# sjpark0905/DNA-LDPC-codes

Measured on AMD Instinct MI355X. Metric: decoded codewords/sec (n=18432, m=2048, 50 BP iters) at 1/2/4/8 GPUs; % HBM roofline, higher is better.
Workload: dtype f64; 1 GPU; bsc-p0.02-100k-per-gpu-bp50; code=decode_n18432_m2048_final.pchk (8,72)-regular, E=147456, input=int8 channel codes in HBM + table code*ln49 (LR = host exp), batch_per_gpu=100000, global_batch=100000, max_iter=50, algo=bp, parallelism=dp1 (contiguous codeword shards, no collective), resident_per_pass=192, group_tiles=3, nontemporal_d=False, continuous=True, resident_pool=True, syndrome_split=False

## Files before the change

dna-ldpc-codes_amd/csrc/engine.hip:

```cpp
#include <hip/hip_ext.h>
#include <hip/hip_runtime.h>

#include <algorithm>
#include <cmath>
#include <cstdio>
#include <cstdlib>
#include <cstring>
#include <thread>
#include <type_traits>
#include <utility>

#include "engine.hpp"
#include "kernels.hpp"
#include "kernels_int.hpp"
#include "encode_kernels.hpp"

namespace ldpc {

static_assert(kTile == dev::TILE && kMsaRecPlanes == dev::MSA_REC_PLANES && kMsaErShift == dev::MSA_ER_SHIFT,
              "engine_plan.hpp restates the kernels' layout constants");
constexpr int kProbes = 4;

static thread_local std::string g_err;
void set_error(const std::string& msg) { g_err = msg; }
// ... 203 lines not shown
int LanePool::check_fault()
{
    if (!h_fault) return LDPC_OK;
    volatile unsigned long long* w = h_fault.get();
    std::string msg;
    for (int k = 1; k < dev::kFaultWords; k++) {
        const unsigned long long v = w[k];
        if (!(v & dev::kFaultTag)) continue;
        w[k] = 0ull;
        if (!msg.empty()) continue;
        int64_t idx = (int64_t)(v & dev::kFaultIndex);
        if (idx & (int64_t)(1ull << 47)) idx -= (int64_t)(1ull << 48);
        if (k == dev::kFaultSchedule)
            msg = "device schedule fault: the code fill of tile " + std::to_string(-1 - idx) +
                  " found live or finished lanes";
        else if (k == dev::kFaultIters)
            msg = "device lane bookkeeping fault: codeword index " + std::to_string(idx) +
                  " out of range for the iteration count / valid flag access";
        else
            msg = "device lane bookkeeping fault: pool slot or codeword index " + std::to_string(idx) +
                  " out of range for " + (k == dev::kFaultOutput ? "a finished codeword's hard bits / posterior" : "a refill's input row");
    }
    if (msg.empty()) return LDPC_OK;
    set_error(msg + " (skipped; the decode's outputs are incomplete)");
    return LDPC_ERR_DEVICE;
}

void LanePool::clear_faults()
{
    volatile unsigned long long* w = h_fault.get();
    for (int k = 1; w && k < dev::kFaultWords; k++) w[k] = 0ull;
}

Engine::~Engine()
{
    if (device >= 0) (void)hipSetDevice(device);
    if (stream) (void)hipStreamSynchronize(stream.get());
}

static double* msa_rec(double* scratch) { return scratch; }
static uint16_t* msa_meta(double* scratch, int64_t tiles, int32_t M)
{
    return reinterpret_cast<uint16_t*>(scratch + (size_t)tiles * M * dev::MSA_REC_PLANES * dev::TILE);
}

template <typename F>
static void with_bools(F&& f)
{
    f();
}
template <typename F, typename... Bs>
static void with_bools(F&& f, bool b, Bs... rest)
{
    if (b) with_bools([&](auto... cs) { f(std::true_type{}, cs...); }, rest...);
    else with_bools([&](auto... cs) { f(std::false_type{}, cs...); }, rest...);
}
template <int... Vs, typename F, typename... Bs>
static bool dispatch(int v, std::integer_sequence<int, Vs...>, F&& f, Bs... bs)
{
    return ((v == Vs && (with_bools([&](auto... cs) { f(std::integral_constant<int, Vs>{}, cs...); }, bs...), true)) || ...);
}

int Engine::init(const HostGraph* graph, int dev, int algorithm, int64_t chunk, const ldpc_schedule* schedule,
                 bool resolved)
{
    g = graph;
    device = dev;
    algo = algorithm;
    if (resolved && schedule && (schedule->flags_set & kResolved)) {
        sched = *schedule;
        sched.pool_tiles = std::max(sched.pool_tiles, 0);
        sched.poll_every = std::max(sched.poll_every, 1);
        sched.syn_blocks = std::min(std::max(sched.syn_blocks, 1), 256);
    } else {
        sched = resolve_schedule(schedule);
    }
    if (algo < LDPC_ALGO_BP || algo > LDPC_ALGO_GALLAGER_B2) { set_error("unknown algorithm"); return LDPC_ERR_ARG; }
    int rc;
    if ((rc = select_device("engine", dev)) || (rc = make_stream(stream))) return rc;
    size_t fr = 0, tot = 0;
    if (chunk <= 0) LDPC_HIP(hipMemGetInfo(&fr, &tot));
    p = plan_engine(*g, algo, chunk, sched, fr);
    if (p.error) { set_error(p.error); return LDPC_ERR_ARG; }

    if ((rc = dg.build(*g, p.msa_c))) return rc;
    if (p.cont && (rc = lp.build(p, g->N))) return rc;
    const size_t E = (size_t)std::max<int64_t>(g->E, 1), cap = (size_t)p.cap, tiles = (size_t)p.cap_tiles, N = (size_t)g->N;
    if ((rc = dev_alloc(v2c, cap * E))) return rc;
    if (!p.res && (rc = dev_alloc(c2v_buf, p.c2v_bytes / sizeof(double)))) return rc;
    if ((rc = dev_alloc(prior, cap * N)) || (p.msa_c && (rc = dev_alloc(d_sgn, cap * N))) ||
        (rc = dev_alloc(hard, tiles * N)) || (rc = dev_alloc(active, tiles)) || (rc = dev_alloc(iters, cap)) ||
        (rc = dev_alloc(valid, cap)))
        return rc;
    if (algo < LDPC_ALGO_QMSA && (p.res || p.group_tiles < p.cap_tiles)) return probe(kProbes);
    return LDPC_OK;
}

int32_t Engine::flags() const
{
    return (p.nt_d ? LDPC_SCHED_NONTEMPORAL : 0) | (p.cont ? LDPC_SCHED_CONTINUOUS : 0) |
           (p.msa_c ? LDPC_SCHED_MSA_COMPRESSED : 0) | (p.res ? LDPC_SCHED_RESIDENT : 0) |
           (p.syn_blocks > 0 ? LDPC_SCHED_SPLIT_SYNDROME : 0) | (p.first_fp ? LDPC_SCHED_FIRST_FROM_PRIOR : 0) |
           (p.handover ? LDPC_SCHED_HANDOVER : 0) | (p.fuse_block >= 0 ? LDPC_SCHED_FUSE_ROW_BLOCK : 0) |
           (sched.flags & (LDPC_SCHED_LR_TABLE | LDPC_SCHED_DEBUG_NO_DRAIN | LDPC_SCHED_DEBUG_BAD_LANE));
}

int Engine::probe(int probes)
{
    dev_ptr<double>& pool = p.res ? v2c : c2v_buf;
    std::vector<dev_ptr<double>> cand;
    cand.push_back(std::move(pool));
    size_t best = 0;
    const int rc = time_candidates(probes, cand, &best);
    pool = std::move(cand[best]);
    return rc;
}

int Engine::time_candidates(int probes, std::vector<dev_ptr<double>>& cand, size_t* best)
{
    const size_t E = (size_t)std::max<int64_t>(g->E, 1);
    const size_t bytes = p.res ? (size_t)p.cap * E * sizeof(double) : p.c2v_bytes;
    const unsigned gt = (unsigned)(p.res ? p.cap_tiles : std::min<int64_t>(p.group_tiles, p.cap_tiles));
    hipStream_t s = stream.get();
    LDPC_HIP(hipMemsetAsync((p.res ? cand[0] : v2c).get(), 0, (size_t)gt * 64 * E * sizeof(double), s));
    LDPC_HIP(hipMemsetAsync(prior.get(), 0, (size_t)gt * 64 * g->N * sizeof(double), s));
    LDPC_HIP(hipMemsetAsync(active.get(), 0xff, (size_t)gt * sizeof(uint64_t), s));
    if (d_sgn) LDPC_HIP(hipMemsetAsync(d_sgn.get(), 0, (size_t)gt * 64 * g->N, s));
    for (int i = 1; i < probes; i++) {
        void* c = nullptr;
        if (hipMalloc(&c, bytes) != hipSuccess) { (void)hipGetLastError(); break; }
        cand.emplace_back(static_cast<double*>(c));
    }
    for (auto& c : cand) LDPC_HIP(hipMemsetAsync(c.get(), 0, bytes, s));
    Event e0, e1;
    int rc;
    if ((rc = make_event(e0, hipEventDefault)) || (rc = make_event(e1, hipEventDefault))) return rc;
    float best_ms = 1e30f;
    for (size_t c = 0; c < cand.size(); c++) {
        if (p.res) std::swap(v2c, cand[c]);
        float ms = 0;
        rc = time_steps((p.res ? v2c : cand[c]).get(), gt, e0.get(), e1.get(), &ms);
        if (p.res) std::swap(v2c, cand[c]);
        if (rc) return rc;
        if (ms < best_ms) { best_ms = ms; *best = c; }
    }
    return LDPC_OK;
}

int Engine::time_steps(double* pool, unsigned gt, hipEvent_t e0, hipEvent_t e1, float* ms)
{
    int rc;
    for (int rep = 0; rep < 5; rep++) {
        if (rep == 1) LDPC_HIP(hipEventRecord(e0, stream.get()));
        if ((rc = launch_check(pool, 0, gt, nullptr, true))) return rc;
        if ((rc = launch_var(pool, 0, gt, nullptr, dev::Refill{}, true))) return rc;
    }
    LDPC_HIP(hipEventRecord(e1, stream.get()));
    LDPC_HIP(hipEventSynchronize(e1));
    LDPC_HIP(hipEventElapsedTime(ms, e0, e1));
    return LDPC_OK;
}

int Engine::launch_check(double* scratch, int64_t t0, unsigned gt, const dev::ResStep* rstep, bool timing)
{
    using namespace dev;
    const int32_t M = g->M;
    const int64_t E = g->E;
    const bool reg72 = g->regular_dc && g->dc_max == 72;
    const dim3 grid((M + 3) / 4, gt), blk(256);
    const bool msa = algo == LDPC_ALGO_MSA;
    const int kc = timing ? K_UNCOUNTED : K_CHECK;
    int rc = LDPC_OK;
    if (rstep && !reg72) {
        const int cb = gen_bucket(g->dc_max, CheckBuckets{});
        if (!p.res || scratch != v2c.get() || t0 != 0 || !cb) { set_error("resident check: bad state"); return LDPC_ERR_ARG; }
        dispatch(cb, CheckBuckets{}, [&](auto D, auto MSA) {
            rc = launch(kc, (k_check_gr_res<MSA(), D()>), grid, blk, v2c, dg.row_ptr, M, E, *rstep);
        }, msa);
        return rc;
    }
    if (rstep) {
        if (!p.res || p.msa_c || scratch != v2c.get()) { set_error("resident check: bad state"); return LDPC_ERR_ARG; }
        if (msa) return launch(kc, (k_check_msa<72, false, true>), grid, blk, v2c, v2c, active, M, E, t0, *rstep);
        if (p.fuse_block >= 0) {
            if (t0 != 0) { set_error("resident check: bad state"); return LDPC_ERR_ARG; }
            const int32_t Q = M / 8;
            return launch(kc, (k_check_bp_skip<72>), grid, blk, v2c, v2c, M, E, p.fuse_block * Q, (p.fuse_block + 1) * Q,
                          *rstep);
        }
        return launch(kc, (k_check_bp<72, false, true>), grid, blk, v2c, v2c, active, M, E, t0, *rstep);
    }
    if (p.msa_c) {
        const dim3 g1((unsigned)((M + 3) / 4) * gt);
        with_bools([&](auto NT) {
            rc = launch(kc, (k_check_msa_c<72, NT()>), g1, blk, v2c, msa_rec(scratch), msa_meta(scratch, p.c2v_tiles, M),
                        active, dg.row_pos, M, E, t0, gt);
        }, p.nt_d);
        return rc;
    }
    if (reg72) {
        with_bools([&](auto NT) {
            if (msa) rc = launch(kc, (k_check_msa<72, NT(), false>), grid, blk, v2c, scratch, active, M, E, t0, ResStep{});
            else rc = launch(kc, (k_check_bp<72, NT(), false>), grid, blk, v2c, scratch, active, M, E, t0, ResStep{});
        }, p.nt_d);
        return rc;
    }
    const bool bp = algo == LDPC_ALGO_BP;
    const bool in_regs = dispatch(gen_bucket(g->dc_max, CheckBuckets{}), CheckBuckets{}, [&](auto D, auto MSA) {
        rc = launch(kc, k_check_gr<MSA(), D()>, grid, blk, v2c, scratch, active, dg.row_ptr, M, E, t0);
    }, !bp);
    if (!in_regs && bp) rc = launch(kc, k_check_bp_gen, grid, blk, v2c, scratch, active, dg.row_ptr, M, E, t0);
    else if (!in_regs) rc = launch(kc, k_check_msa_gen, grid, blk, v2c, scratch, active, dg.row_ptr, M, E, t0);
    return rc;
}

int Engine::var_cpw_for(const dev::Refill& rf) const
{
    if (p.var_cpw > 0) return p.var_cpw;
    return (rf.fresh && rf.in_code && (p.res || p.msa_c)) ? kDefaultVarCpwCoded : kDefaultVarCpw;
}

int Engine::launch_var(double* scratch, int64_t t0, unsigned gt, double* pt, const dev::Refill& rf, bool timing)
{
    using namespace dev;
    const int32_t N = g->N, M = g->M;
    const int64_t E = g->E;
    const bool reg8 = g->regular_dv && g->dv_max == 8;
    const bool cnt = rf.fresh != nullptr;
    const bool pc = cnt && rf.in_code != nullptr;
    const bool inplace = scratch == v2c.get();
    const int kc = timing ? K_UNCOUNTED : K_VAR;
    int rc = LDPC_OK;
    bool ok = true;
    if (p.msa_c) {
        int cpw = std::min(var_cpw_for(rf), 4);
        if (N % (4 * cpw) != 0) cpw = 1;
        const unsigned nb = gt * (unsigned)(N / (4 * cpw));
        const double* rec = msa_rec(scratch);
        const uint16_t* meta = msa_meta(scratch, p.c2v_tiles, M);
        ok = dispatch(cpw, std::integer_sequence<int, 1, 2, 3, 4>{}, [&](auto CPW, auto CONT, auto NT, auto PC) {
            if constexpr (CONT() || !PC())
                rc = launch(kc, (k_var_msa_c<72, 8, CONT(), CPW(), NT(), PC()>), dim3(nb), dim3(256), rec, meta, v2c, prior,
                            hard, d_sgn, active, dg.col_er, pt, N, M, E, t0, (uint32_t)gt, dg.msa_pa, dg.msa_pb, rf);
        }, cnt, p.nt_d, pc);
    } else if (reg8 && p.fuse_block >= 0 && cnt && inplace) {
        if (t0 != 0 || timing) { set_error("fused row block: bad state"); return LDPC_ERR_ARG; }
        const dim3 grid((unsigned)(M / 8), gt);
        with_bools([&](auto PC) {
            rc = launch(kc, (k_var_bp_fused<kFuseWaves, kFuseCpw, PC()>), grid, dim3(64 * kFuseWaves), v2c, prior, hard,
                        active, dg.col_edge, dg.col_idx, pt, N, E, p.fuse_block * (M / 8), rf);
        }, pc);
    } else if (reg8) {
        const int want = var_cpw_for(rf);
        const int cpw = (want != 3 && N % (4 * want) == 0) ? want : 1;
        const dim3 grid((unsigned)((N + 4 * cpw - 1) / (4 * cpw)), gt);
        ok = dispatch(cpw, std::integer_sequence<int, 1, 2, 4, 8>{},
                      [&](auto CPW, auto MSA, auto NT, auto CONT, auto IP, auto PC) {
            if constexpr (!(IP() && NT()) && (CONT() || !PC()))
                rc = launch(kc, (k_var_m<MSA(), 8, NT(), CONT(), CPW(), IP(), PC()>), grid, dim3(256), scratch, v2c, prior,
                            hard, active, dg.col_edge, pt, N, E, t0, rf);
        }, algo == LDPC_ALGO_MSA, p.nt_d && !inplace, cnt, inplace, pc);
    } else {
        const dim3 grid((N + 3) / 4, gt), blk(256);
        const int vb = gen_bucket(g->dv_max, VarBuckets{});
        const bool bp = algo == LDPC_ALGO_BP;
        if (cnt) {
            if (!vb) { set_error("continuous mode needs column degrees <= 32"); return LDPC_ERR_ARG; }
            dispatch(vb, VarBuckets{}, [&](auto D, auto MSA, auto PC, auto IP) {
                rc = launch(kc, (k_var_gr_cont<MSA(), D(), PC(), IP()>), grid, blk, scratch, v2c, prior, hard, active,
                            dg.col_ptr, dg.col_edge, pt, N, E, t0, rf);
            }, algo == LDPC_ALGO_MSA, pc, inplace);
        } else {
            const bool in_regs = dispatch(vb, VarBuckets{}, [&](auto D, auto MSA) {
                rc = launch(kc, k_var_gr<MSA(), D()>, grid, blk, scratch, v2c, prior, hard, active, dg.col_ptr,
                            dg.col_edge, pt, N, E, t0);
            }, !bp);
            if (!in_regs && bp) rc = launch(kc, k_var_bp_gen, grid, blk, scratch, v2c, prior, hard, active, dg.col_ptr, dg.col_edge, pt, N, E, t0);
            else if (!in_regs) rc = launch(kc, k_var_msa_gen, grid, blk, scratch, v2c, prior, hard, active, dg.col_ptr, dg.col_edge, pt, N, E, t0);
        }
    }
    if (!ok) { set_error("variable phase: no kernel for these columns per wave"); return LDPC_ERR_ARG; }
    return rc;
}

template <typename Init, typename Check, typename Var, typename Final>
int Engine::fixed_pass(const DecodeCall& c, Init&& init, Check&& check, Var&& var, Final&& finalize)
{
    using namespace dev;
    const int32_t M = g->M, N = g->N;
    const int64_t Bc = c.B, tiles = (Bc + 63) / 64;
    const bool reg_rowT = g->regular_dc && dg.col_idx_T != nullptr;
    int rc;
    if (c.post && (rc = post_t.ensure((size_t)p.cap * N, stream.get()))) return rc;
    double* pt = c.post ? post_t.get() : nullptr;
    const dim3 blk(256);
    if ((rc = init(tiles))) return rc;
    for (int32_t n = 0;; n++) {
        if (reg_rowT && g->dc_max == 72)
            rc = launch(K_SYN, k_syndrome<72>, dim3((unsigned)tiles), dim3(1024), hard, active, iters, valid, dg.row_ptr,
                        dg.col_idx, dg.col_idx_T, M, N, n, c.max_iter);
        else
            rc = launch(K_SYN, k_syndrome<0>, dim3((unsigned)tiles), dim3(1024), hard, active, iters, valid, dg.row_ptr,
                        dg.col_idx, dg.col_idx_T, M, N, n, c.max_iter);
        if (rc) return rc;
        if (n >= c.max_iter) break;
        for (int64_t t0 = 0; t0 < tiles; t0 += p.group_tiles) {
            const unsigned gt = (unsigned)std::min<int64_t>(p.group_tiles, tiles - t0);
            if ((rc = check(t0, gt)) || (rc = var(t0, gt, n, pt))) return rc;
        }
    }
    if (c.post && (rc = finalize(tiles))) return rc;
    if (c.hard) {
        const int64_t nblk = Bc * ((N + 255) / 256);
        const unsigned grid = (unsigned)std::min<int64_t>(nblk, 1 << 20);
        if ((rc = launch(K_FINAL, k_unpack_hard, dim3(grid), blk, hard, c.hard, Bc, N))) return rc;
    }
    hipStream_t s = stream.get();
    if (c.iters) LDPC_HIP(hipMemcpyAsync(c.iters, iters.get(), (size_t)Bc * sizeof(int32_t), hipMemcpyDeviceToDevice, s));
    if (c.valid) LDPC_HIP(hipMemcpyAsync(c.valid, valid.get(), (size_t)Bc, hipMemcpyDeviceToDevice, s));
    return LDPC_OK;
}

int Engine::run_chunk(const DecodeCall& c)
{
    using namespace dev;
    const int32_t N = g->N;
    const int64_t E = g->E;
    const int msa = algo == LDPC_ALGO_MSA;
    if (msa && c.in_kind == LDPC_IN_LR) { set_error("min-sum takes LLR input"); return LDPC_ERR_ARG; }
    if (msa && c.post_kind == LDPC_POST_RATIO) { set_error("LDPC_POST_RATIO is BP-only"); return LDPC_ERR_ARG; }
    const dim3 blk(256);
    return fixed_pass(
// ... 361 lines not shown
```

dna-ldpc-codes_amd/csrc/kernels.hpp:

```cpp
#pragma once
#include <hip/hip_runtime.h>
#include <cstdint>

#include "kargs.hpp"

namespace ldpc {
namespace dev {

constexpr int TILE = 64;

__device__ __forceinline__ int wave_id() { return __builtin_amdgcn_readfirstlane((int)(threadIdx.x >> 6)); }
__device__ __forceinline__ int lane_id() { return (int)(threadIdx.x & 63); }

__device__ __forceinline__ unsigned xcd_block(unsigned b, unsigned nb)
{
    const unsigned q = nb / 8, r = nb % 8, x = b % 8;
    return (x < r ? x * (q + 1) : r * (q + 1) + (x - r) * q) + b / 8;
}

__device__ __forceinline__ uint64_t shfl_xor_u64(uint64_t v, int m)
{
    uint32_t lo = (uint32_t)v, hi = (uint32_t)(v >> 32);
    lo = (uint32_t)__shfl_xor((int)lo, m);
    hi = (uint32_t)__shfl_xor((int)hi, m);
// ... 657 lines not shown
    bool bad_in = false;
    int bad_v = 0;
    if (fr) {
        const size_t rb = (size_t)refill_row(rf.lane_b[t * TILE + lane], rf, bad_in) * N;
        bad_v = bad_in ? 1 : 0;
#pragma unroll
        for (int c = 0; c < CPW; ++c) {
            if constexpr (PC) kin[c] = rf.in_code[rb + j0 + c];
            else xin[c] = rf.in[rb + j0 + c];
        }
    }
    if (live) {
#pragma unroll
        for (int c = 0; c < CPW; ++c) {
            pv[c] = prior_at<PC>(prior, rf, ((size_t)t * N + j0 + c) * TILE + lane);
#pragma unroll
            for (int s = 0; s < DV; ++s) l[c][s] = c2v_t[(size_t)eid[c][s] * TILE + lane];
        }
    }
    if constexpr (PC) {
        if (fr) {
#pragma unroll
            for (int c = 0; c < CPW; ++c) xin[c] = rf.ptab[kin[c] + kCodeBias];
        }
    }
    if (HO && lastm != 0) {
        const int64_t lb = ls ? rf.pend_b[t * TILE + lane] : 0;
        const bool lok = out_ok(lb, rf);
        uint64_t hwf[CPW];
#pragma unroll
        for (int c = 0; c < CPW; ++c) {
            const bool hf = var_column_final<MSA, DV>(ls, pv[c], l[c], lok, rf, lb, N, j0 + c);
            hwf[c] = __ballot(hf);
            if (lane == 0) rf.hard_fin[(size_t)t * N + j0 + c] = hwf[c];
        }
        if (ls && lok) store_fin_hard<CPW>(rf, hwf, lb, N, j0, lane);
        if (ls && !lok) lane_fault(rf.fault, kFaultOutput, t * TILE + lane);
    }
    const bool fok = out_ok(fb, rf);
    if (CONT && fl && fok) {
        uint64_t hw[CPW];
#pragma unroll
        for (int c = 0; c < CPW; ++c) hw[c] = hard[(size_t)t * N + j0 + c];
        store_fin_hard<CPW>(rf, hw, fb, N, j0, lane);
    }
#pragma unroll
    for (int c = 0; c < CPW; ++c) {
        const int32_t j = j0 + c;
        const size_t pj = ((size_t)t * N + j) * TILE + lane;
        if (CONT && fl && fok && rf.post_out)
            var_column_fin_post<MSA, PC>(rf, prior, post, pj, (size_t)fb * N + j, fn);
        bool h;
        double dv[DV], np;
        var_column<MSA, DV, PC>(live, fr, ls, pv[c], xin[c], l[c], rf, post, pj, dv, np, h);
        if (CONT && fr) {
            if constexpr (PC) rf.pcode[pj] = kin[c];
            else prior[pj] = np;
        }
        const bool skip_init = CONT && rf.prior_only && !live;
        if (!skip_init && (line_occupied(touched, lane) || fr || live)) {
#pragma unroll
            for (int s = 0; s < DV; ++s) st<NT>(v2c + (tb + eid[c][s]) * TILE + lane, dv[s]);
        }
        merge_touched(hard, t, N, j, touched, h, lane);
    }
    if (CONT && fl && !fok) lane_fault(rf.fault, kFaultOutput, t * TILE + lane);
    asm volatile("" : "+v"(bad_v));
    if (bad_v) lane_fault(rf.fault, kFaultRefill, t * TILE + lane);
}

template <bool MSA, int DV, bool NT, bool CONT, int CPW, bool INPLACE, bool PC = false>
__global__ __launch_bounds__(256) void k_var_m(typename Msg<INPLACE>::in c2v, typename Msg<INPLACE>::out v2c,
                                               double* __restrict__ prior, uint64_t* __restrict__ hard,
                                               const uint64_t* __restrict__ active,
                                               const int32_t* __restrict__ col_edge, double* __restrict__ post,
                                               int32_t N, int64_t E, int64_t t0, Refill rf)
{
    static_assert(CONT || !PC, "coded priors come with continuous refills");
    var_m_block<MSA, DV, NT, CONT, CPW, INPLACE, PC>(c2v + (size_t)blockIdx.y * E * TILE, v2c, prior, hard, active,
                                                 col_edge, post, N, E, t0 + blockIdx.y,
                                                 xcd_block(blockIdx.x, gridDim.x), rf);
}

constexpr int kFuseWaves = 8, kFuseCpw = 3;
template <int W, int CPW, bool PC>
__global__ __launch_bounds__(64 * W) void k_var_bp_fused(double* msg, double* __restrict__ prior,
                                                         uint64_t* __restrict__ hard,
                                                         const uint64_t* __restrict__ active,
                                                         const int32_t* __restrict__ col_edge,
                                                         const int32_t* __restrict__ col_idx, double* post, int32_t N,
                                                         int64_t E, int32_t row0, Refill rf)
{
    constexpr int DC = 72, DV = 8, KW = DC / W;
    static_assert(DC % W == 0 && KW % CPW == 0, "the row's columns split evenly over the waves and their rounds");
    __shared__ double sd[DC][TILE];
    const int lane = lane_id(), w = wave_id();
    const int64_t t = blockIdx.y;
    const int32_t row = row0 + (int32_t)xcd_block(blockIdx.x, gridDim.x);
    const uint64_t act = active[t];
    const uint64_t frm = rf.fresh[t];
    const uint64_t touched = act | frm;
    const uint64_t fm = rf.fin ? rf.fin[t] : 0ull;
    const uint64_t lastm = rf.last ? rf.last[t] : 0ull;
    if (touched == 0 && fm == 0) return;
    const bool live = (act >> lane) & 1ull;
    const bool fr = (frm >> lane) & 1ull;
    const bool fl = (fm >> lane) & 1ull;
    const bool ls = (lastm >> lane) & 1ull;
    int64_t fb = 0;
    int32_t fn = 0;
    if (fl) {
        fb = rf.fin_b[t * TILE + lane];
        fn = rf.fin_n[t * TILE + lane];
    }
    double* m_t = msg + (size_t)t * E * TILE;
    const int k0 = w * KW;
    const int32_t e0 = row * DC + k0;
    bool bad_in = false;
    int bad_v = 0;
    size_t rb = 0;
    if (fr) {
        rb = (size_t)refill_row(rf.lane_b[t * TILE + lane], rf, bad_in) * N;
        bad_v = bad_in ? 1 : 0;
    }
    const int64_t lb = ls ? rf.pend_b[t * TILE + lane] : 0;
    const bool lok = out_ok(lb, rf), fok = out_ok(fb, rf);
    const bool keep = line_occupied(touched, lane) || fr || live;
#pragma unroll
    for (int r = 0; r < KW; r += CPW) {
        int32_t j[CPW], eid[CPW][DV];
#pragma unroll
        for (int c = 0; c < CPW; ++c) j[c] = col_idx[e0 + r + c];
#pragma unroll
        for (int c = 0; c < CPW; ++c)
#pragma unroll
            for (int s = 0; s < DV; ++s) eid[c][s] = col_edge[(size_t)j[c] * DV + s];
        double l[CPW][DV], pv[CPW], xin[CPW];
        int8_t kin[CPW];
        if (fr) {
#pragma unroll
            for (int c = 0; c < CPW; ++c) {
                if constexpr (PC) kin[c] = rf.in_code[rb + j[c]];
                else xin[c] = rf.in[rb + j[c]];
            }
        }
        if (live) {
#pragma unroll
            for (int c = 0; c < CPW; ++c) {
                pv[c] = prior_at<PC>(prior, rf, ((size_t)t * N + j[c]) * TILE + lane);
#pragma unroll
                for (int s = 0; s < DV; ++s) l[c][s] = m_t[(size_t)eid[c][s] * TILE + lane];
            }
        }
        if constexpr (PC) {
            if (fr) {
#pragma unroll
                for (int c = 0; c < CPW; ++c) xin[c] = rf.ptab[kin[c] + kCodeBias];
            }
        }
        if (lastm != 0) {
#pragma unroll
            for (int c = 0; c < CPW; ++c) {
                const uint64_t hwf = __ballot(var_column_final<false, DV>(ls, pv[c], l[c], lok, rf, lb, N, j[c]));
                if (lane == 0) rf.hard_fin[(size_t)t * N + j[c]] = hwf;
                if (ls && lok) store_fin_hard<1>(rf, &hwf, lb, N, j[c], lane);
            }
        }
        if (fl && fok) {
#pragma unroll
            for (int c = 0; c < CPW; ++c) {
                const uint64_t hw = hard[(size_t)t * N + j[c]];
                store_fin_hard<1>(rf, &hw, fb, N, j[c], lane);
            }
        }
#pragma unroll
        for (int c = 0; c < CPW; ++c) {
            const size_t pj = ((size_t)t * N + j[c]) * TILE + lane;
            if (fl && fok && rf.post_out) var_column_fin_post<false, PC>(rf, prior, post, pj, (size_t)fb * N + j[c], fn);
            bool h;
            double dv[DV], np;
            var_column<false, DV, PC>(live, fr, ls, pv[c], xin[c], l[c], rf, post, pj, dv, np, h);
            if (fr) {
                if constexpr (PC) rf.pcode[pj] = kin[c];
                else prior[pj] = np;
            }
            const int32_t ea = e0 + r + c;
            if (keep) {
#pragma unroll
                for (int s = 0; s < DV; ++s) {
                    if (eid[c][s] == ea) sd[k0 + r + c][lane] = dv[s];
                    else m_t[(size_t)eid[c][s] * TILE + lane] = dv[s];
                }
            }
            merge_touched(hard, t, N, j[c], touched, h, lane);
        }
    }
    if (lastm != 0 && ls && !lok) lane_fault(rf.fault, kFaultOutput, t * TILE + lane);
    if (fl && !fok) lane_fault(rf.fault, kFaultOutput, t * TILE + lane);
    asm volatile("" : "+v"(bad_v));
    if (bad_v) lane_fault(rf.fault, kFaultRefill, t * TILE + lane);
    __syncthreads();
    if (touched == 0) return;
    double p = 1.0;
    for (int g = 0; g < w; ++g) {
        double y[KW];
#pragma unroll
        for (int i = 0; i < KW; ++i) y[i] = sd[g * KW + i][lane];
#pragma unroll
        for (int i = 0; i < KW; ++i) p = p * y[i];
    }
    double x[KW], pk[KW];
#pragma unroll
    for (int i = 0; i < KW; ++i) x[i] = sd[k0 + i][lane];
#pragma unroll
    for (int i = 0; i < KW; ++i) { pk[i] = p; p = p * x[i]; }
    double sfx = 1.0;
    for (int g = W - 1; g > w; --g) {
        double y[KW];
#pragma unroll
        for (int i = 0; i < KW; ++i) y[i] = sd[g * KW + i][lane];
#pragma unroll
        for (int i = KW - 1; i >= 0; --i) sfx = sfx * y[i];
    }
#pragma unroll
    for (int i = KW - 1; i >= 0; --i) {
        const double tt = pk[i] * sfx;
        if (keep) m_t[(size_t)(e0 + i) * TILE + lane] = (1.0 + tt) / (1.0 - tt);
        sfx = sfx * x[i];
    }
}

__device__ __forceinline__ void merge_hard(uint64_t* __restrict__ hard, int64_t t, int32_t N, int32_t j, uint64_t mask,
                                           bool h, int lane)
{
    const uint64_t m = __ballot(h);
    if (lane == 0 && mask) {
        const size_t o = (size_t)t * N + j;
        const uint64_t old = (mask == ~0ull) ? 0ull : hard[o];
        hard[o] = (old & ~mask) | (m & mask);
    }
}

__global__ __launch_bounds__(256) void k_var_bp_gen(const double* __restrict__ lr, double* __restrict__ dmsg,
                                                    const double* __restrict__ prior, uint64_t* __restrict__ hard,
                                                    const uint64_t* __restrict__ active, const int32_t* __restrict__ col_ptr,
                                                    const int32_t* __restrict__ col_edge, double* __restrict__ post,
                                                    int32_t N, int64_t E, int64_t t0)
{
    const int lane = lane_id();
    const int32_t j = blockIdx.x * 4 + wave_id();
    const int64_t t = t0 + blockIdx.y;
    if (j >= N) return;
    const uint64_t act = active[t];
    if (act == 0) return;
    const bool live = (act >> lane) & 1ull;
    const int32_t a = col_ptr[j], b = col_ptr[j + 1];
    const size_t tb = (size_t)t * E, tl = (size_t)blockIdx.y * E;
    bool h = false;
    if (live) {
        const size_t pj = ((size_t)t * N + j) * TILE + lane;
        double p = prior[pj];
        for (int32_t q = a; q < b; ++q) {
            const int32_t e = col_edge[q];
            dmsg[(tb + e) * TILE + lane] = p;
            p = p * lr[(tl + e) * TILE + lane];
        }
        if (__builtin_isnan(p)) p = 1.0;
        h = (p <= 1.0);
        if (post) post[pj] = p;
        double acc = 1.0;
        for (int32_t q = b - 1; q >= a; --q) {
            const int32_t e = col_edge[q];
            const size_t o = (tb + e) * TILE + lane;
            double v = dmsg[o] * acc;
            if (__builtin_isnan(v)) v = 1.0;
            acc = acc * lr[(tl + e) * TILE + lane];
            dmsg[o] = 1.0 - 2.0 / (1.0 + v);
        }
    }
    merge_hard(hard, t, N, j, act, h, lane);
}

template <int D, bool INPLACE = false>
__device__ __forceinline__ void check_msa_compute_rt(const double (&x)[D], int32_t d, typename Msg<INPLACE>::out dst)
{
    double m1 = __builtin_inf(), m2 = __builtin_inf();
    int32_t i1 = -1;
    uint32_t neg = 0;
#pragma unroll
    for (int k = 0; k < D; ++k) {
        if (k < d) {
            const double av = __builtin_fabs(x[k]);
            neg ^= (x[k] >= 0) ? 0u : 1u;
            if (av < m1) { m1 = av; i1 = k; }
        }
    }
#pragma unroll
    for (int k = 0; k < D; ++k) {
        if (k < d) {
            const double av = __builtin_fabs(x[k]);
            if (k != i1 && av < m2) m2 = av;
        }
    }
    const double a0 = __builtin_fabs(x[0]), a1 = __builtin_fabs(x[1]);
#pragma unroll
    for (int k = 0; k < D; ++k) {
        if (k < d) {
            const double af = (k == 0) ? a1 : a0;
            double mag = (k == i1) ? m2 : m1;
            if (__builtin_isnan(af)) mag = af;
            const uint32_t nk = (x[k] >= 0) ? 0u : 1u;
            const int sign = ((neg ^ nk) & 1u) ? -1 : 1;
// ... 399 lines not shown
    const uint64_t act = active[t];
    const uint64_t frm = rf.fresh[t];
    const uint64_t touched = act | frm;
    const uint64_t fm = rf.fin ? rf.fin[t] : 0ull;
    if (touched == 0 && fm == 0) return;
    const bool live = (act >> lane) & 1ull;
    const bool fr = (frm >> lane) & 1ull;
    const bool fl = (fm >> lane) & 1ull;
    int64_t fb = 0;
    int32_t fn = 0;
    if (fl) {
        fb = rf.fin_b[t * TILE + lane];
        fn = rf.fin_n[t * TILE + lane];
    }
    const int32_t a = col_ptr[j], d = col_ptr[j + 1] - a;
    const size_t tb = (size_t)t * E;
    typename Msg<INPLACE>::in c2v_t = c2v + (size_t)blockIdx.y * E * TILE;
    int32_t eid[D];
#pragma unroll
    for (int s = 0; s < D; ++s)
        if (s < d) eid[s] = col_edge[a + s];
    bool bad_in = false;
    int bad_v = 0;
    double xin = 0.0;
    int8_t kin = 0;
    if (fr) {
        const size_t rb = (size_t)refill_row(rf.lane_b[t * TILE + lane], rf, bad_in) * N;
        bad_v = bad_in ? 1 : 0;
        if constexpr (PC) kin = rf.in_code[rb + j];
        else xin = rf.in[rb + j];
    }
    const size_t pj = ((size_t)t * N + j) * TILE + lane;
    double l[D];
    double pv = 0.0;
    if (live) {
        pv = prior_at<PC>(prior, rf, pj);
#pragma unroll
        for (int s = 0; s < D; ++s)
            if (s < d) l[s] = c2v_t[(size_t)eid[s] * TILE + lane];
    }
    if constexpr (PC) {
        if (fr) xin = rf.ptab[kin + kCodeBias];
    }
    const bool fok = out_ok(fb, rf);
    if (fl && fok) {
        const uint64_t hw[1] = {hard[(size_t)t * N + j]};
        store_fin_hard<1>(rf, hw, fb, N, j, lane);
        if (rf.post_out) {
            const double q = fn > 0 ? post[pj] : prior_at<PC>(prior, rf, pj);
            if (MSA) rf.post_out[(size_t)fb * N + j] = q;
            else {
                const double P = __builtin_isnan(q) ? 1.0 : q;
                rf.post_out[(size_t)fb * N + j] = rf.post_ratio ? P : log(P);
            }
        }
    }
    bool h = false;
    double dv[D];
#pragma unroll
    for (int s = 0; s < D; ++s) dv[s] = 0.0;
    double np = live ? pv : 0.0;
    if (fr) {
        var_refill_init<MSA, D>(xin, !PC && rf.in_is_llr, dv, np, h);
    } else if (live) {
        const auto keep = [&](int s, double v) { dv[s] = v; };
        if constexpr (MSA) var_msa_update<D>(pv, l, d, post, pj, h, keep);
        else var_bp_update<D>(pv, l, d, post, pj, h, keep);
    }
    if (fr) {
        if constexpr (PC) rf.pcode[pj] = kin;
        else prior[pj] = np;
    }
    if (line_occupied(touched, lane) || fr || live) {
#pragma unroll
        for (int s = 0; s < D; ++s)
            if (s < d) v2c[(tb + eid[s]) * TILE + lane] = dv[s];
    }
    merge_hard(hard, t, N, j, touched, h, lane);
    if (fl && !fok) lane_fault(rf.fault, kFaultOutput, t * TILE + lane);
    asm volatile("" : "+v"(bad_v));
    if (bad_v) lane_fault(rf.fault, kFaultRefill, t * TILE + lane);
}

typedef unsigned int u32x2 __attribute__((ext_vector_type(2)));
typedef unsigned int u32x4 __attribute__((ext_vector_type(4)));
constexpr int kBufNT = 2;
__device__ __forceinline__ __amdgpu_buffer_rsrc_t buf_rsrc(const void* base, uint64_t bytes)
{
    return __builtin_amdgcn_make_buffer_rsrc(const_cast<void*>(base), (short)0,
                                            (int)(bytes < 0x7fffffffull ? bytes : 0x7fffffffull), 0x00020000);
}

constexpr int MSA_REC_PLANES = 4;
constexpr uint32_t MSA_META_ID = 0x7fu;
constexpr uint32_t MSA_META_NONE = 0x1000u;

template <int DC, bool NT>
__global__ __launch_bounds__(256) void k_check_msa_c(const double* __restrict__ v2c, double* __restrict__ rec,
                                                     uint16_t* __restrict__ meta, const uint64_t* __restrict__ active,
                                                     const int32_t* __restrict__ row_pos, int32_t M, int64_t E,
                                                     int64_t t0, uint32_t gt)
{
    static_assert(DC >= 2 && DC <= 96, "row degree");
    const int lane = lane_id();
    const uint32_t ty = blockIdx.x % gt;
    const int32_t row = (int32_t)(blockIdx.x / gt) * 4 + wave_id();
    const int64_t t = t0 + ty;
    const uint64_t act = active[t];
    if (!(row < M && line_occupied(act, lane))) return;
    const auto rv2c = buf_rsrc(v2c + (size_t)t * E * TILE, (uint64_t)E * TILE * 8);
    const int32_t* __restrict__ pos = row_pos + (size_t)row * DC;
    double x[DC];
#pragma unroll
    for (int k = 0; k < DC; ++k)
        x[k] = __builtin_bit_cast(double, __builtin_amdgcn_raw_buffer_load_b64(rv2c, lane * 8, pos[k] * (TILE * 8),
                                                                               NT ? kBufNT : 0));
    double m1 = __builtin_inf(), m2 = __builtin_inf();
    int i1 = -1;
    bool neg = false, anynan = false;
#pragma unroll
    for (int k = 0; k < DC; ++k) {
        const double a = __builtin_fabs(x[k]);
        neg ^= !(x[k] >= 0);
        anynan |= __builtin_isnan(a);
        i1 = (a < m1) ? k : i1;
        m2 = __builtin_fmin(m2, __builtin_fmax(m1, a));
        m1 = __builtin_fmin(m1, a);
    }
    if (__builtin_expect(__ballot(anynan) != 0ull, 0) && anynan) {
        m1 = __builtin_inf();
        m2 = __builtin_inf();
        i1 = -1;
#pragma unroll
        for (int k = 0; k < DC; ++k) {
            const double a = __builtin_fabs(x[k]);
            const bool lt1 = a < m1, lt2 = a < m2;
            m2 = lt1 ? m1 : (lt2 ? a : m2);
            m1 = lt1 ? a : m1;
            i1 = lt1 ? k : i1;
        }
    }
    const double a0 = __builtin_fabs(x[0]), a1 = __builtin_fabs(x[1]);
    const bool nan0 = __builtin_isnan(a0), nan1 = __builtin_isnan(a1);
    double* __restrict__ r = rec + ((size_t)ty * M + row) * (MSA_REC_PLANES * TILE) + lane;
    r[0] = m1;
    r[TILE] = m2;
    if (nan0) r[2 * TILE] = a0;
    if (nan1) r[3 * TILE] = a1;
    meta[((size_t)ty * M + row) * TILE + lane] =
        (uint16_t)(((neg ? 1u : 0u) << 15) | ((nan1 ? 1u : 0u) << 14) | ((nan0 ? 1u : 0u) << 13) |
                   (i1 < 0 ? MSA_META_NONE : ((uint32_t)(row * DC + i1) & MSA_META_ID)));
}

__device__ __forceinline__ double flip_sign(double v, uint32_t neg)
{
    return __longlong_as_double(__double_as_longlong(v) ^ ((long long)(neg & 1u) << 63));
}

constexpr int MSA_ER_SHIFT = 18;
constexpr uint32_t MSA_ER_EDGE = (1u << MSA_ER_SHIFT) - 1;
__device__ __forceinline__ uint32_t er_pos(uint32_t er, int DC)
{
    return (er & MSA_ER_EDGE) - (er >> MSA_ER_SHIFT) * (uint32_t)DC;
}

template <int DC, int DV, bool CONT, int CPW, bool NT, bool PC = false>
__global__ __launch_bounds__(256) void k_var_msa_c(const double* __restrict__ rec, const uint16_t* __restrict__ meta,
                                                   double* __restrict__ v2c,
                                                   double* __restrict__ prior, uint64_t* __restrict__ hard,
                                                   uint8_t* __restrict__ sgn, const uint64_t* __restrict__ active,
                                                   const uint32_t* __restrict__ col_er, double* __restrict__ post,
                                                   int32_t N, int32_t M, int64_t E, int64_t t0, uint32_t gt,
                                                   int32_t vpa, int32_t vpb, Refill rf)
{
    const int lane = lane_id();
// ... 339 lines not shown
```

Measured before the change: 28390 codewords/s.

## Software-pipeline fused BP row kernel with load window and buffer intrinsics

Restructures the fused variable/check row kernel to issue edge-message loads for a sliding window of upcoming columns while processing the current one, replacing fixed CPW rounds. Message loads and stores now go through raw buffer intrinsics with 32-bit offsets, and the fused path is disabled when a tile's message plane exceeds 2 GB. A rare-path template variant handles refill and finalisation with window 1, so the common steady-state path avoids those branches. The aim is more memory-level parallelism and cheaper addressing, at the cost of higher register pressure from holding KW columns of state.

After: 28760 codewords/s (median of 6 runs). 1.3% higher.

```diff
diff --git a/dna-ldpc-codes_amd/csrc/engine.hip b/dna-ldpc-codes_amd/csrc/engine.hip
--- a/dna-ldpc-codes_amd/csrc/engine.hip
+++ b/dna-ldpc-codes_amd/csrc/engine.hip
@@ -309,6 +309,7 @@
     if (chunk <= 0) LDPC_HIP(hipMemGetInfo(&fr, &tot));
     p = plan_engine(*g, algo, chunk, sched, fr);
     if (p.error) { set_error(p.error); return LDPC_ERR_ARG; }
+    if (g->E * (int64_t)(dev::TILE * sizeof(double)) > 0x7fffffff) p.fuse_block = -1;
 
     if ((rc = dg.build(*g, p.msa_c))) return rc;
     if (p.cont && (rc = lp.build(p, g->N))) return rc;
@@ -474,7 +475,7 @@
         if (t0 != 0 || timing) { set_error("fused row block: bad state"); return LDPC_ERR_ARG; }
         const dim3 grid((unsigned)(M / 8), gt);
         with_bools([&](auto PC) {
-            rc = launch(kc, (k_var_bp_fused<kFuseWaves, kFuseCpw, PC()>), grid, dim3(64 * kFuseWaves), v2c, prior, hard,
+            rc = launch(kc, (k_var_bp_fused<kFuseWaves, kFuseWindow, PC()>), grid, dim3(64 * kFuseWaves), v2c, prior, hard,
                         active, dg.col_edge, dg.col_idx, pt, N, E, p.fuse_block * (M / 8), rf);
         }, pc);
     } else if (reg8) {
diff --git a/dna-ldpc-codes_amd/csrc/kernels.hpp b/dna-ldpc-codes_amd/csrc/kernels.hpp
--- a/dna-ldpc-codes_amd/csrc/kernels.hpp
+++ b/dna-ldpc-codes_amd/csrc/kernels.hpp
@@ -763,27 +763,30 @@
                                                  xcd_block(blockIdx.x, gridDim.x), rf);
 }
 
-constexpr int kFuseWaves = 8, kFuseCpw = 3;
-template <int W, int CPW, bool PC>
-__global__ __launch_bounds__(64 * W) void k_var_bp_fused(double* msg, double* __restrict__ prior,
-                                                         uint64_t* __restrict__ hard,
-                                                         const uint64_t* __restrict__ active,
-                                                         const int32_t* __restrict__ col_edge,
-                                                         const int32_t* __restrict__ col_idx, double* post, int32_t N,
-                                                         int64_t E, int32_t row0, Refill rf)
-{
-    constexpr int DC = 72, DV = 8, KW = DC / W;
-    static_assert(DC % W == 0 && KW % CPW == 0, "the row's columns split evenly over the waves and their rounds");
-    __shared__ double sd[DC][TILE];
+typedef unsigned int u32x2 __attribute__((ext_vector_type(2)));
+typedef unsigned int u32x4 __attribute__((ext_vector_type(4)));
+constexpr int kBufNT = 2;
+__device__ __forceinline__ __amdgpu_buffer_rsrc_t buf_rsrc(const void* base, uint64_t bytes)
+{
+    return __builtin_amdgcn_make_buffer_rsrc(const_cast<void*>(base), (short)0,
+                                            (int)(bytes < 0x7fffffffull ? bytes : 0x7fffffffull), 0x00020000);
+}
+
+constexpr int kFuseWaves = 8, kFuseWindow = 4;
+constexpr int kFuseDc = 72;
+
+template <int W, int WIN, bool PC, bool RARE>
+__device__ __forceinline__ void var_bp_fused_row(double (&sd)[kFuseDc][TILE], double* msg, double* __restrict__ prior,
+                                                 uint64_t* __restrict__ hard, const int32_t* __restrict__ col_edge,
+                                                 const int32_t* __restrict__ col_idx, double* post, int32_t N,
+                                                 int64_t E, int32_t row, int64_t t, uint64_t act, uint64_t frm_,
+                                                 uint64_t fm_, uint64_t lastm_, const Refill& rf)
+{
+    constexpr int DC = kFuseDc, DV = 8, KW = DC / W;
+    static_assert(DC % W == 0 && WIN >= 1, "the row's columns split evenly over the waves");
     const int lane = lane_id(), w = wave_id();
-    const int64_t t = blockIdx.y;
-    const int32_t row = row0 + (int32_t)xcd_block(blockIdx.x, gridDim.x);
-    const uint64_t act = active[t];
-    const uint64_t frm = rf.fresh[t];
+    const uint64_t frm = RARE ? frm_ : 0ull, fm = RARE ? fm_ : 0ull, lastm = RARE ? lastm_ : 0ull;
     const uint64_t touched = act | frm;
-    const uint64_t fm = rf.fin ? rf.fin[t] : 0ull;
-    const uint64_t lastm = rf.last ? rf.last[t] : 0ull;
-    if (touched == 0 && fm == 0) return;
     const bool live = (act >> lane) & 1ull;
     const bool fr = (frm >> lane) & 1ull;
     const bool fl = (fm >> lane) & 1ull;
@@ -794,7 +797,8 @@
         fb = rf.fin_b[t * TILE + lane];
         fn = rf.fin_n[t * TILE + lane];
     }
-    double* m_t = msg + (size_t)t * E * TILE;
+    const auto rm = buf_rsrc(msg + (size_t)t * E * TILE, (uint64_t)E * TILE * 8);
+    const int lo = lane * 8;
     const int k0 = w * KW;
     const int32_t e0 = row * DC + k0;
     bool bad_in = false;
@@ -807,74 +811,61 @@
     const int64_t lb = ls ? rf.pend_b[t * TILE + lane] : 0;
     const bool lok = out_ok(lb, rf), fok = out_ok(fb, rf);
     const bool keep = line_occupied(touched, lane) || fr || live;
-#pragma unroll
-    for (int r = 0; r < KW; r += CPW) {
-        int32_t j[CPW], eid[CPW][DV];
-#pragma unroll
-        for (int c = 0; c < CPW; ++c) j[c] = col_idx[e0 + r + c];
-#pragma unroll
-        for (int c = 0; c < CPW; ++c)
-#pragma unroll
-            for (int s = 0; s < DV; ++s) eid[c][s] = col_edge[(size_t)j[c] * DV + s];
-        double l[CPW][DV], pv[CPW], xin[CPW];
-        int8_t kin[CPW];
+    int32_t j[KW], eid[KW][DV];
+    double l[KW][DV], pv[KW], xin[KW];
+    int8_t kin[KW];
+#pragma unroll
+    for (int k = 0; k < KW; ++k) j[k] = col_idx[e0 + k];
+    auto issue = [&](int k) __attribute__((always_inline)) {
+#pragma unroll
+        for (int s = 0; s < DV; ++s) eid[k][s] = col_edge[(size_t)j[k] * DV + s];
         if (fr) {
-#pragma unroll
-            for (int c = 0; c < CPW; ++c) {
-                if constexpr (PC) kin[c] = rf.in_code[rb + j[c]];
-                else xin[c] = rf.in[rb + j[c]];
+            if constexpr (PC) kin[k] = rf.in_code[rb + j[k]];
+            else xin[k] = rf.in[rb + j[k]];
+        }
+        if (live) {
+            pv[k] = prior_at<PC>(prior, rf, ((size_t)t * N + j[k]) * TILE + lane);
+#pragma unroll
+            for (int s = 0; s < DV; ++s)
+                l[k][s] = __builtin_bit_cast(double, __builtin_amdgcn_raw_buffer_load_b64(rm, lo, eid[k][s] * (TILE * 8), 0));
+        }
+    };
+#pragma unroll
+    for (int k = 0; k < WIN && k < KW; ++k) issue(k);
+#pragma unroll
+    for (int k = 0; k < KW; ++k) {
+        if constexpr (PC) {
+            if (fr) xin[k] = rf.ptab[kin[k] + kCodeBias];
+        }
+        if (lastm != 0) {
+            const uint64_t hwf = __ballot(var_column_final<false, DV>(ls, pv[k], l[k], lok, rf, lb, N, j[k]));
+            if (lane == 0) rf.hard_fin[(size_t)t * N + j[k]] = hwf;
+            if (ls && lok) store_fin_hard<1>(rf, &hwf, lb, N, j[k], lane);
+        }
+        if (fl && fok) {
+            const uint64_t hw = hard[(size_t)t * N + j[k]];
+            store_fin_hard<1>(rf, &hw, fb, N, j[k], lane);
+        }
+        const size_t pj = ((size_t)t * N + j[k]) * TILE + lane;
+        if (fl && fok && rf.post_out) var_column_fin_post<false, PC>(rf, prior, post, pj, (size_t)fb * N + j[k], fn);
+        bool h;
+        double dv[DV], np;
+        var_column<false, DV, PC>(live, fr, ls, pv[k], xin[k], l[k], rf, post, pj, dv, np, h);
+        if (fr) {
+            if constexpr (PC) rf.pcode[pj] = kin[k];
+            else prior[pj] = np;
+        }
+        const int32_t ea = e0 + k;
+        if (keep) {
+#pragma unroll
+            for (int s = 0; s < DV; ++s) {
+                if (eid[k][s] == ea) sd[k0 + k][lane] = dv[s];
+                else
+                    __builtin_amdgcn_raw_buffer_store_b64(__builtin_bit_cast(u32x2, dv[s]), rm, lo, eid[k][s] * (TILE * 8), 0);
             }
         }
-        if (live) {
-#pragma unroll
-            for (int c = 0; c < CPW; ++c) {
-                pv[c] = prior_at<PC>(prior, rf, ((size_t)t * N + j[c]) * TILE + lane);
-#pragma unroll
-                for (int s = 0; s < DV; ++s) l[c][s] = m_t[(size_t)eid[c][s] * TILE + lane];
-            }
-        }
-        if constexpr (PC) {
-            if (fr) {
-#pragma unroll
-                for (int c = 0; c < CPW; ++c) xin[c] = rf.ptab[kin[c] + kCodeBias];
-            }
-        }
-        if (lastm != 0) {
-#pragma unroll
-            for (int c = 0; c < CPW; ++c) {
-                const uint64_t hwf = __ballot(var_column_final<false, DV>(ls, pv[c], l[c], lok, rf, lb, N, j[c]));
-                if (lane == 0) rf.hard_fin[(size_t)t * N + j[c]] = hwf;
-                if (ls && lok) store_fin_hard<1>(rf, &hwf, lb, N, j[c], lane);
-            }
-        }
-        if (fl && fok) {
-#pragma unroll
-            for (int c = 0; c < CPW; ++c) {
-                const uint64_t hw = hard[(size_t)t * N + j[c]];
-                store_fin_hard<1>(rf, &hw, fb, N, j[c], lane);
-            }
-        }
-#pragma unroll
-        for (int c = 0; c < CPW; ++c) {
-            const size_t pj = ((size_t)t * N + j[c]) * TILE + lane;
-            if (fl && fok && rf.post_out) var_column_fin_post<false, PC>(rf, prior, post, pj, (size_t)fb * N + j[c], fn);
-            bool h;
-            double dv[DV], np;
-            var_column<false, DV, PC>(live, fr, ls, pv[c], xin[c], l[c], rf, post, pj, dv, np, h);
-            if (fr) {
-                if constexpr (PC) rf.pcode[pj] = kin[c];
-                else prior[pj] = np;
-            }
-            const int32_t ea = e0 + r + c;
-            if (keep) {
-#pragma unroll
-                for (int s = 0; s < DV; ++s) {
-                    if (eid[c][s] == ea) sd[k0 + r + c][lane] = dv[s];
-                    else m_t[(size_t)eid[c][s] * TILE + lane] = dv[s];
-                }
-            }
-            merge_touched(hard, t, N, j[c], touched, h, lane);
-        }
+        merge_touched(hard, t, N, j[k], touched, h, lane);
+        if (k + WIN < KW) issue(k + WIN);
     }
     if (lastm != 0 && ls && !lok) lane_fault(rf.fault, kFaultOutput, t * TILE + lane);
     if (fl && !fok) lane_fault(rf.fault, kFaultOutput, t * TILE + lane);
@@ -903,12 +894,42 @@
 #pragma unroll
         for (int i = KW - 1; i >= 0; --i) sfx = sfx * y[i];
     }
+    double lr[KW];
 #pragma unroll
     for (int i = KW - 1; i >= 0; --i) {
         const double tt = pk[i] * sfx;
-        if (keep) m_t[(size_t)(e0 + i) * TILE + lane] = (1.0 + tt) / (1.0 - tt);
+        lr[i] = (1.0 + tt) / (1.0 - tt);
         sfx = sfx * x[i];
     }
+    if (keep) {
+#pragma unroll
+        for (int i = KW - 1; i >= 0; --i)
+            __builtin_amdgcn_raw_buffer_store_b64(__builtin_bit_cast(u32x2, lr[i]), rm, lo, (e0 + i) * (TILE * 8), 0);
+    }
+}
+
+template <int W, int WIN, bool PC>
+__global__ __launch_bounds__(64 * W) void k_var_bp_fused(double* msg, double* __restrict__ prior,
+                                                         uint64_t* __restrict__ hard,
+                                                         const uint64_t* __restrict__ active,
+                                                         const int32_t* __restrict__ col_edge,
+                                                         const int32_t* __restrict__ col_idx, double* post, int32_t N,
+                                                         int64_t E, int32_t row0, Refill rf)
+{
+    __shared__ double sd[kFuseDc][TILE];
+    const int64_t t = blockIdx.y;
+    const int32_t row = row0 + (int32_t)xcd_block(blockIdx.x, gridDim.x);
+    const uint64_t act = active[t];
+    const uint64_t frm = rf.fresh[t];
+    const uint64_t fm = rf.fin ? rf.fin[t] : 0ull;
+    const uint64_t lastm = rf.last ? rf.last[t] : 0ull;
+    if ((act | frm) == 0 && fm == 0) return;
+    if ((frm | fm | lastm) != 0)
+        var_bp_fused_row<W, 1, PC, true>(sd, msg, prior, hard, col_edge, col_idx, post, N, E, row, t, act, frm, fm, lastm,
+                                         rf);
+    else
+        var_bp_fused_row<W, WIN, PC, false>(sd, msg, prior, hard, col_edge, col_idx, post, N, E, row, t, act, 0ull, 0ull,
+                                            0ull, rf);
 }
 
 __device__ __forceinline__ void merge_hard(uint64_t* __restrict__ hard, int64_t t, int32_t N, int32_t j, uint64_t mask,
@@ -1474,15 +1495,6 @@
     if (bad_v) lane_fault(rf.fault, kFaultRefill, t * TILE + lane);
 }
 
-typedef unsigned int u32x2 __attribute__((ext_vector_type(2)));
-typedef unsigned int u32x4 __attribute__((ext_vector_type(4)));
-constexpr int kBufNT = 2;
-__device__ __forceinline__ __amdgpu_buffer_rsrc_t buf_rsrc(const void* base, uint64_t bytes)
-{
-    return __builtin_amdgcn_make_buffer_rsrc(const_cast<void*>(base), (short)0,
-                                            (int)(bytes < 0x7fffffffull ? bytes : 0x7fffffffull), 0x00020000);
-}
-
 constexpr int MSA_REC_PLANES = 4;
 constexpr uint32_t MSA_META_ID = 0x7fu;
 constexpr uint32_t MSA_META_NONE = 0x1000u;
```
